# theOehrly/Formula-VAD

Measured on AMD Instinct MI355X. Metric: 48 kHz 480-sample VAD frames/sec whole node; max concurrent real-time streams, higher is better.
Workload: dtype f32

## Files before the change

formula-vad_amd/csrc/fvad_device.h:

```cpp
#pragma once
#pragma clang fp contract(off)
#include <hip/hip_runtime.h>

#include <cmath>

#include "fvad_internal.h"

namespace fvad {

constexpr float kWs = 1.f / 256;

__device__ __forceinline__ float2 cmul(float2 a, float2 b) {
  float2 m;
  m.x = a.x * b.x - a.y * b.y;
  m.y = a.x * b.y + a.y * b.x;
  return m;
}
__device__ __forceinline__ float2 cadd(float2 a, float2 b) { return make_float2(a.x + b.x, a.y + b.y); }
__device__ __forceinline__ float2 csub(float2 a, float2 b) { return make_float2(a.x - b.x, a.y - b.y); }

__device__ __forceinline__ float tansig(const float *__restrict__ table, float x) {
  if (!(x < 8)) return 1;
  if (!(x > -8)) return -1;
  if (x != x) return 0;
  float sign = 1;
  if (x < 0) {
    x = -x;
    sign = -1;
  }
  const int i = (int)floorf(.5f + 25 * x);
  x -= .04f * i;
  float y = table[i];
  const float dy = 1 - y * y;
  y = y + x * dy * (1 - y * x);
  return sign * y;
}
__device__ __forceinline__ float sigmoid(const float *__restrict__ table, float x) {
  return (float)(.5 + .5 * (double)tansig(table, (float)(.5 * (double)x)));
}
__device__ __forceinline__ float activate(const float *__restrict__ table, int act, float x) {
  if (act == kActSigmoid) return sigmoid(table, x);
  if (act == kActTanh) return tansig(table, x);
  return x < 0 ? 0 : x;
}

__device__ __forceinline__ void bfly4(float2 *F, int m, float2 tw1, float2 tw2, float2 tw3) {
  float2 a0 = F[0];
  const float2 s0 = cmul(F[m], tw1), s1 = cmul(F[2 * m], tw2), s2 = cmul(F[3 * m], tw3);
  const float2 s5 = csub(a0, s1);
  a0 = cadd(a0, s1);
  const float2 s3 = cadd(s0, s2), s4 = csub(s0, s2);
  F[2 * m] = csub(a0, s3);
  a0 = cadd(a0, s3);
  F[0] = a0;
  F[m] = make_float2(s5.x + s4.y, s5.y - s4.x);
  F[3 * m] = make_float2(s5.x - s4.y, s5.y + s4.x);
}

__device__ __forceinline__ void bfly3(float2 *F, int m, float2 tw1, float2 tw2, float2 epi3) {
  float2 a0 = F[0];
  const float2 s1 = cmul(F[m], tw1), s2 = cmul(F[2 * m], tw2);
  const float2 s3 = cadd(s1, s2);
  float2 s0 = csub(s1, s2);
  const float2 b1 = make_float2(a0.x - s3.x * .5f, a0.y - s3.y * .5f);
  s0.x *= epi3.y;
  s0.y *= epi3.y;
  a0 = cadd(a0, s3);
  F[0] = a0;
  F[2 * m] = make_float2(b1.x + s0.y, b1.y - s0.x);
  F[m] = make_float2(b1.x - s0.y, b1.y + s0.x);
}

__device__ __forceinline__ void kbfly5(float2 *F, int m, float2 t1, float2 t2, float2 t3, float2 t4, float2 ya,
                                       float2 yb) {
  const float2 s0 = F[0];
  const float2 s1 = cmul(F[m], t1), s2 = cmul(F[2 * m], t2), s3 = cmul(F[3 * m], t3), s4 = cmul(F[4 * m], t4);
  const float2 s7 = cadd(s1, s4), s10 = csub(s1, s4), s8 = cadd(s2, s3), s9 = csub(s2, s3);
  F[0] = make_float2(s0.x + (s7.x + s8.x), s0.y + (s7.y + s8.y));
  const float2 s5 = make_float2(s0.x + s7.x * ya.x + s8.x * yb.x, s0.y + s7.y * ya.x + s8.y * yb.x);
  const float2 s6 = make_float2(s10.y * ya.y + s9.y * yb.y, -(s10.x * ya.y) - s9.x * yb.y);
  F[m] = csub(s5, s6);
  F[4 * m] = cadd(s5, s6);
  const float2 s11 = make_float2(s0.x + s7.x * yb.x + s8.x * ya.x, s0.y + s7.y * yb.x + s8.y * ya.x);
  const float2 s12 = make_float2(-(s10.y * yb.y) + s9.y * ya.y, s10.x * yb.y - s9.x * ya.y);
  F[2 * m] = cadd(s11, s12);
  F[3 * m] = csub(s11, s12);
}

__device__ __forceinline__ void kiss_stage(float2 *W, float2 *S, int p, int m, int nc,
                                           const float2 *__restrict__ tw, int tid, int nt) {
  if (p == 1) return;
  const int fstride = nc / (p * m);
  if (p <= 5) {
    const int nb = fstride * m;
    for (int idx = tid; idx < nb; idx += nt) {
      const int g = idx / m, u = idx - g * m;
      float2 *F = W + g * p * m + u;
      if (p == 4) {
        bfly4(F, m, tw[u * fstride], tw[2 * u * fstride], tw[3 * u * fstride]);
      } else if (p == 2) {
        const float2 t = cmul(F[m], tw[u * fstride]);
        F[m] = csub(F[0], t);
        F[0] = cadd(F[0], t);
      } else if (p == 3) {
        bfly3(F, m, tw[u * fstride], tw[2 * u * fstride], tw[fstride * m]);
      } else {
        kbfly5(F, m, tw[u * fstride], tw[2 * u * fstride], tw[3 * u * fstride], tw[4 * u * fstride],
               tw[fstride * m], tw[fstride * 2 * m]);
      }
    }
    return;
  }
  const int no = fstride * m * p;
  for (int idx = tid; idx < no; idx += nt) {
    const int g = idx / (p * m), r = idx - g * (p * m), q1 = r / m, u = r - q1 * m;
    const float2 *F = W + g * p * m + u;
    const int k = u + q1 * m;
    float2 acc = F[0];
    int twidx = 0;
    for (int q = 1; q < p; q++) {
      twidx += fstride * k;
      if (twidx >= nc) twidx -= nc;
      acc = cadd(acc, cmul(F[q * m], tw[twidx]));
    }
    S[g * p * m + k] = acc;
  }
}

__device__ __forceinline__ void kiss_stages(float2 *W, float2 *S, const int *__restrict__ fac, int nf, int nc,
                                            const float2 *__restrict__ tw, int tid, int nt) {
  for (int k = nf - 1; k >= 0; k--) {
    const int p = fac[2 * k], m = fac[2 * k + 1];
    kiss_stage(W, S, p, m, nc, tw, tid, nt);
    __syncthreads();
    if (p > 5) {
      for (int i = tid; i < nc; i += nt) W[i] = S[i];
      __syncthreads();
    }
  }
}


__device__ __forceinline__ void bfly5(float2 *F, int m, float2 t1, float2 t2, float2 t3, float2 t4, float2 ya,
                                      float2 yb) {
  const float2 s0 = F[0];
  const float2 s1 = cmul(F[m], t1), s2 = cmul(F[2 * m], t2), s3 = cmul(F[3 * m], t3), s4 = cmul(F[4 * m], t4);
  const float2 s7 = cadd(s1, s4), s10 = csub(s1, s4), s8 = cadd(s2, s3), s9 = csub(s2, s3);
  float2 f0;
  f0.x = s0.x + (s7.x + s8.x);
  f0.y = s0.y + (s7.y + s8.y);
  float2 s5, s6, s11, s12;
  s5.x = s0.x + s7.x * ya.x + s8.x * yb.x;
  s5.y = s0.y + s7.y * ya.x + s8.y * yb.x;
  s6.x = s10.y * ya.y + s9.y * yb.y;
  s6.y = -(s10.x * ya.y) - s9.x * yb.y;
  s11.x = s0.x + s7.x * yb.x + s8.x * ya.x;
  s11.y = s0.y + s7.y * yb.x + s8.y * ya.x;
  s12.x = -(s10.y * yb.y) + s9.y * ya.y;
  s12.y = s10.x * yb.y - s9.x * ya.y;
  F[0] = f0;
  F[m] = csub(s5, s6);
  F[4 * m] = cadd(s5, s6);
  F[2 * m] = cadd(s11, s12);
  F[3 * m] = csub(s11, s12);
}

template <int NT>
__device__ void fft960_stages(float2 *W, const float2 *__restrict__ tw, int tid) {
  for (int b = tid; b < 240; b += NT) {
    float2 *F = W + 4 * b;
    float2 f0 = F[0];
    const float2 f1 = F[1], f2 = F[2], f3 = F[3];
    const float2 s0 = csub(f0, f2);
    f0 = cadd(f0, f2);
    float2 s1 = cadd(f1, f3);
    F[2] = csub(f0, s1);
    F[0] = cadd(f0, s1);
    s1 = csub(f1, f3);
    F[1] = make_float2(s0.x + s1.y, s0.y - s1.x);
    F[3] = make_float2(s0.x - s1.y, s0.y + s1.x);
  }
  __syncthreads();
  for (int q = tid; q < 240; q += NT) {
    const int i = q >> 2, j = q & 3;
    bfly4(W + i * 16 + j, 4, tw[j * 60], tw[j * 120], tw[j * 180]);
  }
  __syncthreads();
  for (int q = tid; q < 240; q += NT) {
    const int i = q >> 4, j = q & 15;
    bfly4(W + i * 64 + j, 16, tw[j * 15], tw[j * 30], tw[j * 45]);
  }
  __syncthreads();
  {
    const float2 epi3 = tw[320];
    for (int q = tid; q < 320; q += NT) {
      const int i = q >> 6, k = q & 63;
      bfly3(W + i * 192 + k, 64, tw[k * 5], tw[k * 10], epi3);
    }
  }
  __syncthreads();
  {
    const float2 ya = tw[192], yb = tw[384];
    for (int u = tid; u < 192; u += NT) bfly5(W + u, 192, tw[u], tw[2 * u], tw[3 * u], tw[4 * u], ya, yb);
  }
  __syncthreads();
}

struct Fft960Tw {
  float2 s2[3], s3[3], s4a[2], s4b[2], s5[4];
  float2 epi3, ya, yb;
};
__device__ __forceinline__ void fft960_load(Fft960Tw &t, const float2 *__restrict__ tw, int tid) {
  const int j2 = tid & 3, j3 = tid & 15, k4 = tid & 63;
  t.s2[0] = tw[j2 * 60];
  t.s2[1] = tw[j2 * 120];
  t.s2[2] = tw[j2 * 180];
  t.s3[0] = tw[j3 * 15];
  t.s3[1] = tw[j3 * 30];
  t.s3[2] = tw[j3 * 45];
  t.s4a[0] = tw[k4 * 5];
  t.s4a[1] = tw[k4 * 10];
  t.s4b[0] = t.s4a[0];
  t.s4b[1] = t.s4a[1];
  const int u = tid < 192 ? tid : 0;
  t.s5[0] = tw[u];
  t.s5[1] = tw[2 * u];
  t.s5[2] = tw[3 * u];
  t.s5[3] = tw[4 * u];
  t.epi3 = tw[320];
  t.ya = tw[192];
  t.yb = tw[384];
}
template <int F, int P>
__device__ __forceinline__ void fft960_run(const Fft960Tw &t, float2 (*W)[P], int tid) {
  if (tid < 240) {
#pragma unroll
    for (int fr = 0; fr < F; fr++) {
      float2 *Fp = W[fr] + 4 * tid;
      float2 f0 = Fp[0];
      const float2 f1 = Fp[1], f2 = Fp[2], f3 = Fp[3];
      const float2 s0 = csub(f0, f2);
      f0 = cadd(f0, f2);
      float2 s1 = cadd(f1, f3);
      Fp[2] = csub(f0, s1);
      Fp[0] = cadd(f0, s1);
      s1 = csub(f1, f3);
      Fp[1] = make_float2(s0.x + s1.y, s0.y - s1.x);
      Fp[3] = make_float2(s0.x - s1.y, s0.y + s1.x);
    }
  }
  __syncthreads();
  if (tid < 240) {
#pragma unroll
    for (int fr = 0; fr < F; fr++) bfly4(W[fr] + (tid >> 2) * 16 + (tid & 3), 4, t.s2[0], t.s2[1], t.s2[2]);
  }
  __syncthreads();
  if (tid < 240) {
#pragma unroll
    for (int fr = 0; fr < F; fr++) bfly4(W[fr] + (tid >> 4) * 64 + (tid & 15), 16, t.s3[0], t.s3[1], t.s3[2]);
  }
  __syncthreads();
#pragma unroll
  for (int fr = 0; fr < F; fr++) {
    bfly3(W[fr] + (tid >> 6) * 192 + (tid & 63), 64, t.s4a[0], t.s4a[1], t.epi3);
    if (tid < 64) bfly3(W[fr] + ((tid + 256) >> 6) * 192 + (tid & 63), 64, t.s4b[0], t.s4b[1], t.epi3);
  }
  __syncthreads();
  if (tid < 192) {
#pragma unroll
    for (int fr = 0; fr < F; fr++) bfly5(W[fr] + tid, 192, t.s5[0], t.s5[1], t.s5[2], t.s5[3], t.ya, t.yb);
  }
  __syncthreads();
}

struct BandEdges {
  float frac[400];
  int of[400];
  int e4[kBands + 2];
};
struct BandTab : BandEdges {
  float dct[kBands * kBands];
};
__device__ __forceinline__ void bandedges_load(BandEdges &b, const Plan *__restrict__ P, int tid, int nt) {
  for (int i = tid; i < 400; i += nt) {
    b.frac[i] = P->band_frac[i];
    b.of[i] = P->band_of[i];
  }
  for (int i = tid; i < kBands; i += nt) b.e4[i] = P->eband4[i];
}
__device__ __forceinline__ void bandtab_load(BandTab &b, const Plan *__restrict__ P, int tid, int nt) {
  bandedges_load(b, P, tid, nt);
  for (int i = tid; i < kBands * kBands; i += nt) b.dct[i] = P->dct[i];
}
__device__ __forceinline__ float band_sum_t(const float2 *A, const float2 *B, const BandEdges &T, int b) {
  float acc = 0;
  if (b >= 1) {
#pragma unroll 4
    for (int k = T.e4[b - 1]; k < T.e4[b]; k++) {
      float tmp = A[k].x * B[k].x;
      tmp += A[k].y * B[k].y;
      acc += T.frac[k] * tmp;
    }
  }
  if (b <= kBands - 2) {
#pragma unroll 4
    for (int k = T.e4[b]; k < T.e4[b + 1]; k++) {
      float tmp = A[k].x * B[k].x;
      tmp += A[k].y * B[k].y;
      acc += (1 - T.frac[k]) * tmp;
    }
  }
  if (b == 0 || b == kBands - 1) acc *= 2;
  return acc;
}
__device__ __forceinline__ void band_terms(float2 A, float2 B, const BandEdges &T, int k, float &lo, float &hi) {
  float tmp = A.x * B.x;
  tmp += A.y * B.y;
  hi = T.frac[k] * tmp;
  lo = (1 - T.frac[k]) * tmp;
}
__device__ __forceinline__ float band_chain(const float *lo, const float *hi, const BandEdges &T, int b) {
  float acc = 0;
  if (b >= 1) {
    const float4 *h4 = reinterpret_cast<const float4 *>(hi);
    for (int q = T.e4[b - 1] >> 2; q < T.e4[b] >> 2; q++) {
      const float4 v = h4[q];
      acc += v.x;
      acc += v.y;
      acc += v.z;
      acc += v.w;
    }
  }
  if (b <= kBands - 2) {
    const float4 *l4 = reinterpret_cast<const float4 *>(lo);
    for (int q = T.e4[b] >> 2; q < T.e4[b + 1] >> 2; q++) {
      const float4 v = l4[q];
      acc += v.x;
      acc += v.y;
      acc += v.z;
      acc += v.w;
    }
  }
  if (b == 0 || b == kBands - 1) acc *= 2;
  return acc;
}

__device__ __forceinline__ float interp_gain_t(const float *bandE, const BandEdges &T, int k) {
  if (k >= 400) return 0.0f;
  const int b = T.of[k];
  const float frac = T.frac[k];
  return (1 - frac) * bandE[b] + frac * bandE[b + 1];
}

__device__ __forceinline__ float band_sum(const float2 *A, const float2 *B, const Plan *__restrict__ P, int b) {
  float acc = 0;
  if (b >= 1) {
#pragma unroll 4
    for (int k = P->eband4[b - 1]; k < P->eband4[b]; k++) {
      float tmp = A[k].x * B[k].x;
      tmp += A[k].y * B[k].y;
      acc += P->band_frac[k] * tmp;
    }
  }
  if (b <= kBands - 2) {
#pragma unroll 4
    for (int k = P->eband4[b]; k < P->eband4[b + 1]; k++) {
      float tmp = A[k].x * B[k].x;
      tmp += A[k].y * B[k].y;
      acc += (1 - P->band_frac[k]) * tmp;
    }
  }
  if (b == 0 || b == kBands - 1) acc *= 2;
  return acc;
}

__device__ __forceinline__ float interp_gain(const float *bandE, const Plan *__restrict__ P, int k) {
  if (k >= 400) return 0.0f;
  const int b = P->band_of[k];
  const float frac = P->band_frac[k];
  return (1 - frac) * bandE[b] + frac * bandE[b + 1];
}

__device__ __forceinline__ float dot_seq(float acc, const float *a, int sa, const float *b, int sb, int n) {
  float a0[4], b0[4], a1[4], b1[4];
#pragma unroll
  for (int u = 0; u < 4; u++) {
    a0[u] = a[u * sa];
    b0[u] = b[u * sb];
    a1[u] = a[(4 + u) * sa];
    b1[u] = b[(4 + u) * sb];
  }
  int i = 0;
  for (; i + 8 < n; i += 4) {
    float a2[4], b2[4];
#pragma unroll
    for (int u = 0; u < 4; u++) {
      a2[u] = a[(i + 8 + u) * sa];
      b2[u] = b[(i + 8 + u) * sb];
    }
#pragma unroll
    for (int u = 0; u < 4; u++) acc = acc + a0[u] * b0[u];
#pragma unroll
    for (int u = 0; u < 4; u++) {
      a0[u] = a1[u];
      b0[u] = b1[u];
      a1[u] = a2[u];
      b1[u] = b2[u];
    }
  }
#pragma unroll
  for (int u = 0; u < 4; u++) acc = acc + a0[u] * b0[u];
#pragma unroll
  for (int u = 0; u < 4; u++) acc = acc + a1[u] * b1[u];
  return acc;
}

__device__ void syy_sequence(const float *y, int ys, int len, int max_pitch, float *syy) {
  float Syy = dot_seq(1.0f, y, ys, y, ys, len);
#pragma unroll 4
  for (int i = 0; i < max_pitch; i++) {
    syy[i] = Syy;
    const float ya = y[(i + len) * ys], yb = y[i * ys];
    Syy += ya * ya - yb * yb;
    Syy = (1 > Syy) ? 1 : Syy;
  }
}

__device__ __forceinline__ void best_pitch_visit(float xc, float Syy, int i, float &bn0, float &bn1, float &bd0,
                                                 float &bd1, int *best) {
  float xcorr16 = xc;
  xcorr16 *= 1e-12f;
  const float num = xcorr16 * xcorr16;
  const bool c1 = (xc > 0) && (num * bd1 > bn1 * Syy);
  const bool c2 = c1 && (num * bd0 > bn0 * Syy);
  bn1 = c2 ? bn0 : (c1 ? num : bn1);
  bd1 = c2 ? bd0 : (c1 ? Syy : bd1);
  best[1] = c2 ? best[0] : (c1 ? i : best[1]);
  bn0 = c2 ? num : bn0;
  bd0 = c2 ? Syy : bd0;
  best[0] = c2 ? i : best[0];
}

__device__ __forceinline__ float pitch_gain(float xy, float xx, float yy) { return xy / sqrtf(1 + xx * yy); }

__device__ __forceinline__ int second_check(int k) { return (int)((0x4d54d35534c0ull >> (3 * k)) & 7); }

template <int NT>
__device__ void dense_layer(const DevDense &d, const float *in, float *out, const float *tansig_tab, int tid) {
  for (int i = tid; i < d.nout; i += NT) {
    float sum = d.b[i];
#pragma unroll 8
    for (int j = 0; j < d.nin; j++) sum += d.w[j * d.nout + i] * in[j];
    out[i] = activate(tansig_tab, d.act, kWs * sum);
  }
}

template <int NT>
__device__ void gru_gates(const DevGru &g, const float *in, const float *state, float *zr, const float *tab,
                          int tid) {
  const int N = g.nout, M = g.nin, S3 = 3 * N;
  for (int t = tid; t < 2 * N; t += NT) {
    const int col = t;
    float sum = g.b[col];
#pragma unroll 8
    for (int j = 0; j < M; j++) sum += g.win[j * S3 + col] * in[j];
#pragma unroll 8
    for (int j = 0; j < N; j++) sum += g.wrec[j * S3 + col] * state[j];
    zr[t] = sigmoid(tab, kWs * sum);
  }
}
template <int NT>
__device__ void gru_out(const DevGru &g, const float *in, const float *state, const float *zr, float *h,
                        const float *tab, int tid) {
  const int N = g.nout, M = g.nin, S3 = 3 * N;
  for (int i = tid; i < N; i += NT) {
    float sum = g.b[2 * N + i];
#pragma unroll 8
    for (int j = 0; j < M; j++) sum += g.win[j * S3 + 2 * N + i] * in[j];
#pragma unroll 8
    for (int j = 0; j < N; j++) sum += g.wrec[j * S3 + 2 * N + i] * state[j] * zr[N + j];
    sum = activate(tab, g.act, kWs * sum);
    h[i] = zr[i] * state[i] + (1 - zr[i]) * sum;
  }
}


}
```

formula-vad_amd/csrc/fvad_internal.h:

```cpp
#pragma once
#include <cstddef>
#include <cstdint>

namespace fvad {

constexpr int kFrame = 480;
constexpr int kWin = 960;
constexpr int kFreq = 481;
constexpr int kBands = 22;
constexpr int kFeat = 42;
constexpr int kCeps = 8;
constexpr int kPitchBuf = 1728;
constexpr int kPitchMax = 768;
constexpr int kPitchMin = 60;
constexpr int kXlp = kPitchBuf / 2;
constexpr int kMaxNeurons = 128;
constexpr int kMaxCh = 8;
constexpr int kMaxBandCfg = 4;

constexpr int kMaxFftB = 16384;
constexpr int kMaxFftSize = 1 << 22;
constexpr int kMaxFactors = 32;

constexpr int windows_per_tick(int fft_size) { return fft_size >= kFrame ? 1 : (fft_size - 1 + kFrame) / fft_size; }

namespace st {
constexpr int kPitch = 0;
constexpr int kNdSamples = kPitch;
constexpr int kSyn = kPitch + kPitchBuf;
constexpr int kCepsMem = kSyn + kFrame;
constexpr int kLastG = kCepsMem + kCeps * kBands;
constexpr int kVadGru = kLastG + kBands;
constexpr int kNoiseGru = kVadGru + kMaxNeurons;
constexpr int kDenGru = kNoiseGru + kMaxNeurons;
constexpr int kHp = kDenGru + kMaxNeurons;
constexpr int kMemId = kHp + 2;
constexpr int kLastPeriod = kMemId + 1;
constexpr int kLastGain = kLastPeriod + 1;
constexpr int kFramesDone = kLastGain + 1;
constexpr int kVolAcc = kFramesDone + 1;
constexpr int kCepsDist = kVolAcc + 1;
constexpr int kWords = ((kCepsDist + kCeps * kCeps + 63) / 64) * 64;
}

namespace rnnimg {
constexpr int kMats = 9;
constexpr int kCols[kMats] = {24, 48, 24, 96, 48, 192, 96, 22, 1};
constexpr int kKin[kMats] = {42, 24, 24, 90, 90, 114, 114, 96, 24};
constexpr int kK[kMats] = {42, 48, 48, 138, 138, 210, 210, 96, 24};
constexpr int kSegs[kMats][4] = {{42, 0, 0, 0},   {24, 24, 0, 0},  {24, 24, 0, 0},
                                 {24, 24, 42, 48}, {24, 24, 42, 48}, {24, 48, 42, 96},
                                 {24, 48, 42, 96}, {96, 0, 0, 0},   {24, 0, 0, 0}};
constexpr int pad8(int x) { return (x + 7) & ~7; }
constexpr int pad16(int x) { return (x + 15) & ~15; }
constexpr int seg_off(int m, int g) {
  int o = 0;
  for (int i = 0; i < g; i++) o += pad8(kSegs[m][i]);
  return o;
}
constexpr int stride(int m) { return seg_off(m, 4); }
constexpr int off_b(int m) {
  int o = 0;
  for (int i = 0; i < m; i++) o += pad16(kCols[i]) + pad16(kCols[i] * stride(i));
  return o;
}
constexpr int off_w(int m) { return off_b(m) + pad16(kCols[m]); }
constexpr int kBytes = off_b(kMats);
}

struct Plan {
  float half_window[kFrame];
  float dct[kBands * kBands];
  float tansig[201];
  float band_frac[400];
  int band_of[400];
  int eband4[kBands];
  float tw960[2 * kWin];
  int bitrev960[kWin];
  int ibitrev960[kWin];
  int nfft_b;
  int ncfft_b;
  int stages_b;
  int nfac_b;
  int fac_b[2 * kMaxFactors];
  int generic_b;
  float norm_b;
  float twb[2 * kMaxFftB / 2];
  float superb[2 * kMaxFftB / 4];
  int permb[kMaxFftB / 2];
  float hannb[kMaxFftB];
};

struct DevDense {
  int nin, nout, act;
  const float *w;
  const float *b;
};
struct DevGru {
  int nin, nout, act;
  const float *win;
  const float *wrec;
  const float *b;
};
struct DevModel {
  DevDense in_dense, den_out, vad_out;
  DevGru vad, noise, den;
};

constexpr int kActTanh = 0, kActSigmoid = 1, kActRelu = 2;

struct HostLayer {
  int nin = 0, nout = 0, act = 0;
  bool gru = false;
  std::size_t off_w = 0, off_r = 0, off_b = 0;
};
struct HostModel {
  HostLayer layers[6];
  int8_t *blob = nullptr;
  std::size_t blob_size = 0;
};

void build_plan(Plan *p, int nfft_b);
float build_fftb_tables(int nfft_b, const int *fac, float *twb, float *superb, int *permb, float *hannb);

}

int fvad_synth_group(uint32_t base, int s0, int ns, int n_channels, int total_ticks, int tick0, int n_ticks,
                     float *out, std::size_t out_streams);
```

formula-vad_amd/csrc/fvad_plan.cpp:

```cpp
#include <cmath>
#include <cstdio>
#include <cstdlib>
#include <cstring>

#include "fvad_internal.h"

namespace fvad {
namespace {

const int kEband5ms[kBands] = {0, 1, 2, 3, 4, 5, 6, 7, 8, 10, 12, 14, 16, 20, 24, 28, 34, 40, 48, 60, 78, 100};

void celt_digit_reverse(int fout, int *f, int fstride, const int *factors) {
  const int p = factors[0], m = factors[1];
  if (m == 1) {
    for (int j = 0; j < p; j++) {
      *f = fout + j;
      f += fstride;
    }
  } else {
    for (int j = 0; j < p; j++) {
      celt_digit_reverse(fout, f, fstride * p, factors + 2);
      f += fstride;
      fout += m;
    }
  }
}

void kiss_factor(int n, int *fac, int *nf) {
  int p = 4, k = 0;
  const double floor_sqrt = std::floor(std::sqrt((double)n));
  do {
    while (n % p) {
      switch (p) {
        case 4: p = 2; break;
        case 2: p = 3; break;
        default: p += 2; break;
      }
      if (p > floor_sqrt) p = n;
    }
    n /= p;
    fac[2 * k] = p;
    fac[2 * k + 1] = n;
    k++;
  } while (n > 1);
  *nf = k;
}

void kiss_leaf_perm(int *perm, int out_base, int in_base, int fstride, const int *factors) {
  const int p = factors[0], m = factors[1];
  if (m == 1) {
    for (int j = 0; j < p; j++) perm[out_base + j] = in_base + j * fstride;
  } else {
    for (int j = 0; j < p; j++) kiss_leaf_perm(perm, out_base + j * m, in_base + j * fstride, fstride * p, factors + 2);
  }
}

}

void build_plan(Plan *p, int nfft_b) {
  std::memset(p, 0, sizeof(Plan));
  const double pi = 3.14159265358979323846;
  for (int i = 0; i < kFrame; i++) {
    const double s = std::sin(.5 * pi * (i + .5) / kFrame);
    p->half_window[i] = (float)std::sin(.5 * pi * s * s);
  }
  for (int i = 0; i < kBands; i++)
    for (int j = 0; j < kBands; j++) {
      float v = (float)std::cos((i + .5) * j * pi / kBands);
      if (j == 0) v = (float)(v * std::sqrt(.5));
      p->dct[i * kBands + j] = v;
    }
  for (int i = 0; i < 201; i++) {
    char buf[64];
    std::snprintf(buf, sizeof buf, "%f", std::tanh(0.04 * i));
    p->tansig[i] = std::strtof(buf, nullptr);
  }
  for (int b = 0; b < kBands; b++) p->eband4[b] = kEband5ms[b] << 2;
  for (int b = 0; b < kBands - 1; b++) {
    const int size = (kEband5ms[b + 1] - kEband5ms[b]) << 2;
    for (int j = 0; j < size; j++) {
      p->band_of[(kEband5ms[b] << 2) + j] = b;
      p->band_frac[(kEband5ms[b] << 2) + j] = (float)j / size;
    }
  }
  for (int i = 0; i < kWin; i++) {
    const double cpi = 3.14159265358979323846264338327;
    const double phase = (-2 * cpi / kWin) * i;
    p->tw960[2 * i] = (float)std::cos(phase);
    p->tw960[2 * i + 1] = (float)std::sin(phase);
  }
  const int celt_factors[10] = {5, 192, 3, 64, 4, 16, 4, 4, 4, 1};
  celt_digit_reverse(0, p->bitrev960, 1, celt_factors);
  for (int i = 0; i < kWin; i++) p->ibitrev960[p->bitrev960[i]] = i;
  p->nfft_b = nfft_b;
  p->ncfft_b = nfft_b / 2;
  const int nc = p->ncfft_b;
  kiss_factor(nc, p->fac_b, &p->nfac_b);
  int st = 0;
  for (int i = 0; i < p->nfac_b; i++) {
    st = (p->fac_b[2 * i] == 4 && st == i) ? st + 1 : st;
    if (p->fac_b[2 * i] > 5) p->generic_b = 1;
  }
  p->stages_b = st == p->nfac_b ? st : 0;
  if (nfft_b <= kMaxFftB) p->norm_b = build_fftb_tables(nfft_b, p->fac_b, p->twb, p->superb, p->permb, p->hannb);
}

float build_fftb_tables(int nfft_b, const int *fac, float *twb, float *superb, int *permb, float *hannb) {
  const double pi = 3.14159265358979323846;
  const int nc = nfft_b / 2;
  for (int i = 0; i < nc; i++) {
    const double kpi = 3.141592653589793238462643383279502884197169399375105820974944;
    const double phase = -2 * kpi * i / nc;
    twb[2 * i] = (float)std::cos(phase);
    twb[2 * i + 1] = (float)std::sin(phase);
  }
  for (int i = 0; i < nc / 2; i++) {
    const double phase = -3.14159265358979323846264338327 * ((double)(i + 1) / nc + .5);
    superb[2 * i] = (float)std::cos(phase);
    superb[2 * i + 1] = (float)std::sin(phase);
  }
  kiss_leaf_perm(permb, 0, 0, 1, fac);
  const float N = (float)nfft_b;
  const float two_pi = (float)(2.0 * pi);
  for (int i = 0; i < nfft_b; i++) {
    const float nn = (float)i;
    float acc = 0;
    for (int k = 0; k <= 1; k++) {
      const float kk = (float)k;
      const float sgn = k == 0 ? 1.0f : -1.0f;
      const float arg = ((two_pi * kk) * nn) / N;
      acc += (sgn * 0.5f) * (float)std::cos((double)arg);
    }
    hannb[i] = acc;
  }
  float sum = 0;
  for (int i = 0; i < nfft_b; i++) sum += hannb[i];
  const float window_norm = (float)nfft_b / sum;
  return window_norm / (float)(nfft_b / 2);
}

}
```

formula-vad_amd/csrc/fvad_wave.hip:

```cpp
#pragma clang fp contract(off)
#include <hip/hip_runtime.h>

#include <algorithm>
#include <cmath>

#include "fvad_device.h"
#include "fvad_internal.h"
#include "fvad_staged.h"
#include "fvad_staged_dev.h"
#include "fvad_wavedev.h"
#include "fvad_wfft.h"

namespace fvad {

constexpr int kWB = 8;
constexpr int kWNW = 4;
constexpr int kWOcc = 3;

constexpr int kWaveStatic = (1 << kWavePspec) | (1 << kWaveSynth);
__device__ __forceinline__ bool wave_is_static(const StagedArgs &, WaveKernel k) { return (kWaveStatic >> k) & 1; }
template <int NW = kWNW>
__device__ __forceinline__ long long wave_first(const StagedArgs &a, WaveKernel k, int slot, int lane) {
  return wave_is_static(a, k) ? (long long)blockIdx.x * NW + (threadIdx.x >> 6) : wave_take(a, slot, lane);
}
template <int NW = kWNW>
__device__ __forceinline__ long long wave_next(const StagedArgs &a, WaveKernel k, int slot, int lane, long long g) {
  return wave_is_static(a, k) ? g + (long long)gridDim.x * NW : wave_take(a, slot, lane);
}

__device__ __forceinline__ int batch_frames(const StagedArgs &a, long long g, int lane) {
  return lane < kWB ? frame_of(a, g, kWB, lane) : -1;
}
__device__ __forceinline__ int lane_val(int v, int l) { return __builtin_amdgcn_readlane(v, l); }
__device__ __forceinline__ void settle(int v) { asm volatile("" ::"v"(v)); }

__global__ void __launch_bounds__(64 * kWNW, kWOcc) k_fftAw(StagedArgs a) {
  __shared__ __attribute__((aligned(16))) float2 Rg[kWNW][wfft::kSlots];
  __shared__ WaveTabs tb;
  __shared__ float exb[kWNW][kWB][kBands + 2], lyb[kWNW][kWB][kBands + 2];
  __shared__ int silb[kWNW][kWB];
  const int tid = threadIdx.x, lane = tid & 63, wv = tid >> 6;
  wave_tabs_load(tb, a.plan, tid, 64 * kWNW);
  wfft::Tw tw;
  wfft::load_tw(tw, reinterpret_cast<const float2 *>(a.plan->tw960), lane);
  __syncthreads();
  const BandTab &T = tb.T;
  float2 *R = Rg[wv];
  float *tr = reinterpret_cast<float *>(R);
  const long long nb = ((long long)a.n_streams * a.V + kWB - 1) / kWB;
  for (long long g = wave_first(a, kWaveFftA, kWorkFftA, lane); g < nb; g = wave_next(a, kWaveFftA, kWorkFftA, lane, g)) {
    const int fl = batch_frames(a, g, lane);
    for (int fr = 0; fr < kWB; fr++) {
      const int f = lane_val(fl, fr);
      if (f < 0) continue;
      float2 v[16];
      const float *pb = frame_pb(a, f);
      static_assert(kXlp - kXlpHist == 4 * 60 && kHist % 4 == 0, "x_lp lanes");
      float xm = 0;
      float4 qa = make_float4(0, 0, 0, 0), qb = qa;
      if (lane < 60) {
        const float *q = pb + kHist + 8 * lane;
        xm = q[-1];
        qa = *reinterpret_cast<const float4 *>(q);
        qb = *reinterpret_cast<const float4 *>(q + 4);
      }
      WinRaw w;
      win_load(w, pb + (kPitchBuf - kWin), lane);
      win_apply(w, tb.hw, lane, v);
      wfft::run(v, tw, tb.tw, R, lane);
      float2 *X = a.X + (size_t)f * kFreq;
#pragma unroll
      for (int r = 0; r < 8; r++)
        if (64 * r + lane < kFreq) X[64 * r + lane] = v[r];
      if (lane < 60) {
        float4 o;
        o.x = xlp_value(xm, qa.x, qa.y);
        o.y = xlp_value(qa.y, qa.z, qa.w);
        o.z = xlp_value(qa.w, qb.x, qb.y);
        o.w = xlp_value(qb.y, qb.z, qb.w);
        *reinterpret_cast<float4 *>(frame_xlp(a, f) + kXlpHist + 4 * lane) = o;
      }
#pragma unroll
      for (int r = 0; r < 7; r++) {
        const int n = 64 * r + lane;
        if (n < 400) band_terms(v[r], v[r], T, n, tr[n], tr[400 + n]);
      }
      wfft::wsync();
      if (lane < kBands) {
        const float ex = band_chain(tr, tr + 400, T, lane);
        a.Ex[(size_t)f * kBands + lane] = ex;
        exb[wv][fr][lane] = ex;
        lyb[wv][fr][lane] = (float)log10(1e-2 + (double)ex);
      }
      wfft::wsync();
    }
    if (lane < kWB) {
      const int f = fl;
      if (f >= 0) {
        float *Ly = lyb[wv][lane];
        const float *Exl = exb[wv][lane];
        float logMax = -2, follow = -2, E = 0;
        for (int i = 0; i < kBands; i++) {
          const float ly0 = Ly[i];
          const double bb = (follow - 1.5 > (double)ly0) ? follow - 1.5 : (double)ly0;
          const double aa = ((double)(logMax - 7) > bb) ? (double)(logMax - 7) : bb;
          const float ly = (float)aa;
          Ly[i] = ly;
          logMax = (logMax > ly) ? logMax : ly;
          follow = (float)((follow - 1.5 > (double)ly) ? follow - 1.5 : (double)ly);
          E += Exl[i];
        }
        const int sil = ((double)E < 0.04) ? 1 : 0;
        silb[wv][lane] = sil;
        a.silence[f] = sil;
      }
    }
    wfft::wsync();
    for (int idx = lane; idx < kWB * kBands; idx += 64) {
      const int fr = idx / kBands, b = idx - fr * kBands;
      const int f = __shfl(fl, fr);
      if (f >= 0 && !silb[wv][fr]) {
        const float *Ly = lyb[wv][fr];
        float sum = 0;
#pragma unroll
        for (int j = 0; j < kBands; j++) sum += Ly[j] * T.dct[j * kBands + b];
        float val = (float)(sum * sqrt(2. / 22));
        if (b == 0) val -= 12;
        if (b == 1) val -= 4;
        a.Lyf[(size_t)f * kBands + b] = val;
      }
    }
    wfft::wsync();
  }
}

constexpr int kPNW = 8;
__global__ void __launch_bounds__(64 * kPNW, 4) k_pspecw(StagedArgs a) {
  __shared__ __attribute__((aligned(16))) float2 Rg[kPNW][wfft::kSlots];
  __shared__ WaveTabs tb;
  const int tid = threadIdx.x, lane = tid & 63, wv = tid >> 6;
  wave_tabs_load(tb, a.plan, tid, 64 * kPNW);
  wfft::Tw tw;
  wfft::load_tw(tw, reinterpret_cast<const float2 *>(a.plan->tw960), lane);
  __syncthreads();
  float2 *R = Rg[wv];
  const long long nb = ((long long)a.n_streams * a.V + kWB - 1) / kWB;
  for (long long g = wave_first<kPNW>(a, kWavePspec, kWorkPspec, lane); g < nb;
       g = wave_next<kPNW>(a, kWavePspec, kWorkPspec, lane, g)) {
    const int fl = batch_frames(a, g, lane);
    const int pl = fl >= 0 ? a.pitch[fl] : 0;
    settle(pl);
#pragma unroll 1
    for (int fr = 0; fr < kWB; fr++) {
      const int f = lane_val(fl, fr);
      if (f < 0) continue;
      const float v34 = pspec_frame(a, f, lane_val(pl, fr), tb, tw, R, lane);
      if (lane < 7) a.f34[(size_t)f * 8 + lane] = v34;
    }
  }
}

constexpr int kSNW = 8;
constexpr int kSOcc = 4;
struct SynthTabs {
  BandEdges T;
  wfft::TwTab tw;
  float hw[kFrame];
};
__global__ void __launch_bounds__(64 * kSNW, kSOcc) k_synthw(StagedArgs a) {
  __shared__ __attribute__((aligned(16))) float2 Rg[kSNW][wfft::kSlots];
  __shared__ SynthTabs tb;
  __shared__ float bp[kSNW][3][kBands + 2];
  const int tid = threadIdx.x, lane = tid & 63, wv = tid >> 6;
  bandedges_load(tb.T, a.plan, tid, 64 * kSNW);
  wfft::load_twtab(tb.tw, reinterpret_cast<const float2 *>(a.plan->tw960), tid, 64 * kSNW);
  for (int i = tid; i < kFrame; i += 64 * kSNW) tb.hw[i] = a.plan->half_window[i];
  wfft::Tw tw;
  wfft::load_tw(tw, reinterpret_cast<const float2 *>(a.plan->tw960), lane);
  __syncthreads();
  const BandEdges &T = tb.T;
  float2 *R = Rg[wv];
  float *tr = reinterpret_cast<float *>(R);
  float *rr = bp[wv][0], *nrm = bp[wv][1], *gsm = bp[wv][2];
  const long long nb = ((long long)a.n_streams * a.V + kWB - 1) / kWB;
  for (long long g = wave_first<kSNW>(a, kWaveSynth, kWorkSynth, lane); g < nb;
       g = wave_next<kSNW>(a, kWaveSynth, kWorkSynth, lane, g)) {
    const int fl = batch_frames(a, g, lane);
    const int sl = fl >= 0 ? a.silence[fl] : 0;
    settle(sl);
    for (int fr = 0; fr < kWB; fr++) {
      const int f = lane_val(fl, fr);
      if (f < 0) continue;
      const bool fil = !lane_val(sl, fr);
      const float2 *X = a.X + (size_t)f * kFreq;
      const float2 *P = a.P + (size_t)f * kFreq;
      float2 xv[8], pv[8];
#pragma unroll
      for (int r = 0; r < 8; r++) xv[r] = X[min(64 * r + lane, kFreq - 1)];
#pragma unroll
      for (int r = 0; r < 8; r++) pv[r] = P[min(64 * r + lane, kFreq - 1)];
      const size_t o = (size_t)f * kBands + min(lane, kBands - 1);
      const float Exp = a.Exp[o], Ex = a.Ex[o], Ep = a.Ep[o];
      const float gg = a.gr[o], gs = a.gs[o];
      if (fil) {
        if (lane < kBands) {
          float r;
          if (Exp > gg)
            r = 1;
          else
            r = (float)((double)((Exp * Exp) * (1 - (gg * gg))) / (.001 + (double)((gg * gg) * (1 - (Exp * Exp)))));
          float cl = (0 > r) ? 0 : r;
          cl = (1 < cl) ? 1 : cl;
          r = (float)sqrt((double)cl);
          r = (float)((double)r * sqrt((double)Ex / (1e-8 + (double)Ep)));
          rr[lane] = r;
          gsm[lane] = gs;
        }
        wfft::wsync();
#pragma unroll
        for (int r = 0; r < 8; r++) {
          const int n = 64 * r + lane;
          if (n < kFreq) {
            const float rf = interp_gain_t(rr, T, n);
            xv[r].x += rf * pv[r].x;
            xv[r].y += rf * pv[r].y;
            if (n < 400) band_terms(xv[r], xv[r], T, n, tr[n], tr[400 + n]);
          }
        }
        wfft::wsync();
        if (lane < kBands) {
          const float newE = band_chain(tr, tr + 400, T, lane);
          nrm[lane] = (float)sqrt((double)Ex / (1e-8 + (double)newE));
        }
        wfft::wsync();
#pragma unroll
        for (int r = 0; r < 8; r++) {
          const int n = 64 * r + lane;
          if (n < kFreq) {
            const float nf = interp_gain_t(nrm, T, n);
            xv[r].x *= nf;
            xv[r].y *= nf;
            const float gf = interp_gain_t(gsm, T, n);
            xv[r].x *= gf;
            xv[r].y *= gf;
          }
        }
      }
#pragma unroll
      for (int r = 0; r < 8; r++)
        if (64 * r + lane < kFreq) R[64 * r + lane] = xv[r];
      wfft::wsync();
      float2 v[16];
#pragma unroll
      for (int k = 0; k < 16; k++) {
        const int i = wfft::in_index(lane, k);
        float2 val = make_float2(0, 0);
        if (lane < 60) {
          if (i < kFreq) {
            val = R[i];
          } else {
            const float2 c = R[kWin - i];
            val = make_float2(c.x, -c.y);
          }
        }
        v[k] = make_float2(kScale960 * val.x, kScale960 * val.y);
      }
      wfft::wsync();
      wfft::run(v, tw, tb.tw, R, lane);
      float *y = a.ys + (size_t)f * kWin;
#pragma unroll
      for (int r = 0; r < 15; r++) {
        const int n = 64 * r + lane;
        const int i = (n == 0) ? 0 : kWin - n;
        const float yv = kWin * v[r].x;
        y[i] = yv * win960(tb.hw, i);
      }
      wfft::wsync();
    }
  }
}

constexpr int kFbSlots = 1040;
constexpr int kFbMag = 256;

struct FbTabs {
  float2 t4[4][3][16];
  float2 t5[4][3][64];
};

struct FbTw {
  float2 s2[4][3], s3[3], tw0;
};
__device__ __forceinline__ void fftb_tabs_load(FbTabs &tb, const Plan *__restrict__ P, int tid, int nt) {
  const float2 *__restrict__ twb = reinterpret_cast<const float2 *>(P->twb);
  for (int i = tid; i < 4 * 3 * 16; i += nt) {
    const int d2 = i / 48, r = (i / 16) % 3, u = i % 16;
    tb.t4[d2][r][u] = twb[4 * (r + 1) * (u + 16 * d2)];
  }
  for (int i = tid; i < 4 * 3 * 64; i += nt) {
    const int d3 = i / 192, r = (i / 64) % 3, l = i % 64;
    tb.t5[d3][r][l] = twb[(r + 1) * (l + 64 * d3)];
  }
}
__device__ __forceinline__ void fftb_tw_load(FbTw &w, const Plan *__restrict__ P, int lane) {
  const float2 *__restrict__ twb = reinterpret_cast<const float2 *>(P->twb) + opaque0();
#pragma unroll
  for (int d0 = 0; d0 < 4; d0++)
#pragma unroll
    for (int r = 0; r < 3; r++) w.s2[d0][r] = twb[64 * (r + 1) * d0];
#pragma unroll
  for (int r = 0; r < 3; r++) w.s3[r] = twb[16 * (r + 1) * (lane >> 2)];
  w.tw0 = twb[0];
}

__device__ __forceinline__ float fftb_bands(float2 (&v)[16], float2 *R, float *mag, const FbTabs &tb,
                                            const StagedArgs &a, int lane) {
  const Plan *__restrict__ P = a.plan;
  FbTw w;
  fftb_tw_load(w, P, lane);
  const float2 *__restrict__ sup = reinterpret_cast<const float2 *>(P->superb);
  const int nb = a.n_bands, lo = a.bin_lo_all, hi = a.bin_hi_all;
#pragma unroll
  for (int d1 = 0; d1 < 4; d1++) {
    float2 F[4] = {v[d1], v[d1 + 4], v[d1 + 8], v[d1 + 12]};
    bfly4(F, 1, w.tw0, w.tw0, w.tw0);
#pragma unroll
    for (int u = 0; u < 4; u++) v[d1 + 4 * u] = F[u];
  }
#pragma unroll
  for (int d0 = 0; d0 < 4; d0++) {
    float2 F[4] = {v[4 * d0], v[4 * d0 + 1], v[4 * d0 + 2], v[4 * d0 + 3]};
    bfly4(F, 1, w.s2[d0][0], w.s2[d0][1], w.s2[d0][2]);
#pragma unroll
    for (int u = 0; u < 4; u++) v[4 * d0 + u] = F[u];
  }
  wfft::wsync();
  {
    float2 *wr = R + (lane & 3) + 260 * ((lane >> 2) & 3) + 64 * (lane >> 4);
#pragma unroll
    for (int r = 0; r < 16; r++) wr[4 * (r >> 2) + 16 * (r & 3)] = v[r];
  }
  wfft::wsync();
  {
    const float2 *rd = R + lane;
#pragma unroll
    for (int r = 0; r < 16; r++) v[r] = rd[64 * (r & 3) + 260 * (r >> 2)];
  }
#pragma unroll
  for (int d3 = 0; d3 < 4; d3++) {
    float2 F[4] = {v[4 * d3], v[4 * d3 + 1], v[4 * d3 + 2], v[4 * d3 + 3]};
    bfly4(F, 1, w.s3[0], w.s3[1], w.s3[2]);
#pragma unroll
    for (int u = 0; u < 4; u++) v[4 * d3 + u] = F[u];
  }
#pragma unroll
  for (int d2 = 0; d2 < 4; d2++) {
    float2 F[4] = {v[d2], v[d2 + 4], v[d2 + 8], v[d2 + 12]};
    const int u16 = lane >> 2;
    bfly4(F, 1, tb.t4[d2][0][u16], tb.t4[d2][1][u16], tb.t4[d2][2][u16]);
#pragma unroll
    for (int u = 0; u < 4; u++) v[d2 + 4 * u] = F[u];
  }
  wfft::wsync();
  {
    float2 *wr = R + (lane >> 2) + 260 * (lane & 3);
#pragma unroll
    for (int r = 0; r < 16; r++) wr[16 * (r & 3) + 64 * (r >> 2)] = v[r];
  }
  wfft::wsync();
  {
    const float2 *rd = R + lane;
#pragma unroll
    for (int r = 0; r < 16; r++) v[r] = rd[64 * (r & 3) + 260 * (r >> 2)];
  }
#pragma unroll
  for (int d3 = 0; d3 < 4; d3++) {
    float2 F[4] = {v[d3], v[d3 + 4], v[d3 + 8], v[d3 + 12]};
    bfly4(F, 1, tb.t5[d3][0][lane], tb.t5[d3][1][lane], tb.t5[d3][2][lane]);
#pragma unroll
    for (int u = 0; u < 4; u++) v[d3 + 4 * u] = F[u];
  }
  wfft::wsync();
#pragma unroll
  for (int r = 0; r < 16; r++) R[64 * r + lane] = v[r];
  wfft::wsync();
  const int nc = 1024;
  for (int k = lo + lane; k <= hi; k += 64) {
    float re, imv;
    if (k == 0) {
      re = R[0].x + R[0].y;
      imv = 0;
    } else if (k == nc) {
      re = R[0].x - R[0].y;
      imv = 0;
    } else {
      const int kk = (k < nc / 2) ? k : nc - k;
      const float2 fpk = R[kk];
      const float2 fpnk = make_float2(R[nc - kk].x, -R[nc - kk].y);
      const float2 f1k = cadd(fpk, fpnk), f2k = csub(fpk, fpnk);
      const float2 tw2 = cmul(f2k, sup[kk - 1]);
      if (k < nc / 2) {
        re = (f1k.x + tw2.x) * ((float).5);
        imv = (f1k.y + tw2.y) * ((float).5);
      } else {
        re = (f1k.x - tw2.x) * ((float).5);
        imv = (tw2.y - f1k.y) * ((float).5);
      }
    }
    const float r2 = re * re, i2 = imv * imv;
    mag[k - lo] = sqrtf(r2 + i2) * P->norm_b;
  }
  wfft::wsync();
  float acc = 0.0f;
  if (lane < nb)
    for (int k = a.band_lo[lane]; k <= a.band_hi[lane]; k++) acc += mag[k - lo];
  wfft::wsync();
  return acc;
}

__global__ void __launch_bounds__(64 * kWNW, kWOcc) k_fftbw(StagedArgs a) {
  __shared__ __attribute__((aligned(16))) float2 Rg[kWNW][kFbSlots];
  __shared__ float mg[kWNW][kFbMag];
  __shared__ FbTabs tb;
  const int tid = threadIdx.x, lane = tid & 63, wv = tid >> 6;
  const Plan *__restrict__ P = a.plan;
  fftb_tabs_load(tb, P, tid, 64 * kWNW);
  __syncthreads();
  float2 *R = Rg[wv];
  float *mag = mg[wv];
  const int C = a.n_channels, nb = a.n_bands;
  const long long items = (long long)a.n_streams * a.wmax * C;
  const long long nw = (long long)gridDim.x * kWNW;
  for (long long it = (long long)blockIdx.x * kWNW + wv; it < items; it += nw) {
    const int c = (int)(it % C);
    const long long sj = it / C;
    const int s = (int)(sj / a.wmax), j = (int)(sj - (long long)s * a.wmax);
    const int t = a.win_tick[(size_t)s * a.wmax + j];
    if (t < 0) continue;
    const long long wstart = a.win_start[(size_t)s * a.wmax + j];
    const float *ring = a.ring + ((size_t)s * C + c) * a.ring_len;
    const int rl = a.ring_len, w0 = (int)(wstart % rl);
    float2 v[16];
#pragma unroll
    for (int r = 0; r < 16; r++) {
      const int k = lane + 64 * r;
      int i0 = w0 + 2 * k;
      i0 -= (i0 >= rl) ? rl : 0;
      int i1 = i0 + 1;
      i1 -= (i1 >= rl) ? rl : 0;
      const float t0 = ring[i0] * P->hannb[2 * k];
      const float t1 = ring[i1] * P->hannb[2 * k + 1];
      v[r] = make_float2(t0, t1);
    }
    const float band = fftb_bands(v, R, mag, tb, a, lane);
    if (lane < nb) a.out_band[(((size_t)t * a.n_streams + s) * C + c) * nb + lane] = band;
  }
}

__global__ void __launch_bounds__(64 * kWNW, kWOcc) k_olafb(StagedArgs a) {
  __shared__ __attribute__((aligned(16))) float2 Rg[kWNW][kFbSlots];
  __shared__ float mg[kWNW][kFbMag];
  __shared__ float ovg[kWNW][kFrame];
  __shared__ FbTabs tb;
  const int tid = threadIdx.x, lane = tid & 63, wv = tid >> 6;
  const Plan *__restrict__ P = a.plan;
  fftb_tabs_load(tb, P, tid, 64 * kWNW);
  __syncthreads();
  constexpr int FB = 2048;
  float *ov = ovg[wv];
  static_assert(kFbSlots * 2 >= FB, "window fits the exchange region");
  float2 *R = Rg[wv];
  float *W = reinterpret_cast<float *>(R);
  float *mag = mg[wv];
  const int C = a.n_channels, nb = a.n_bands, B = a.n_streams, V = a.V;
  const int G = kWNW / C;
  const int wvu = __builtin_amdgcn_readfirstlane(wv);
  const int sw = wvu / C, c = wvu - sw * C;
  const float kInv = a.raw_s16 ? 1.0f : 1.0f / (float)32767;
  const int rl = a.ring_len;
  for (int sb = blockIdx.x * G; sb < B; sb += gridDim.x * G) {
    const int s = sb + sw;
    const bool on = sw < G && s < B;
    const int nt = __builtin_amdgcn_readfirstlane(on ? ticks_of(a, s) : 0);
    float *stp = a.state + (size_t)(on ? s : 0) * st::kWords;
    int fd0 = 0;
    float vol = 0;
    if (nt > 0) {
      fd0 = __builtin_amdgcn_readfirstlane(reinterpret_cast<const int *>(stp)[st::kFramesDone]);
      vol = __int_as_float(__builtin_amdgcn_readfirstlane(__float_as_int(stp[st::kVolAcc])));
    }
    long long ws = (long long)fd0 * kFrame / FB * FB;
    const float *ring = a.ring + ((size_t)(on ? s : 0) * C + c) * rl;
    if (nt > 0) {
      const int ncarry = (int)((long long)fd0 * kFrame - ws);
      const int r0 = (int)(ws % rl);
      for (int i = lane; i < ncarry; i += 64) {
        int ri = r0 + i;
        ri -= ri >= rl ? rl : 0;
        W[i] = ring[ri];
      }
    }
    __syncthreads();
    if (nt > 0) {
      const float *ysr = a.ys + (size_t)s * V * kWin;
      const bool sl = lane < 60;
      const int q = 8 * lane;
      auto load = [&](int t, float4 (&cur)[2], float4 (&prv)[2]) {
        const int v = t * C + c;
        const float *cp = ysr + (size_t)v * kWin + q;
        const float *pp = v == 0 ? stp + st::kSyn + q : ysr + (size_t)(v - 1) * kWin + kFrame + q;
        if (sl) {
          cur[0] = *reinterpret_cast<const float4 *>(cp);
          cur[1] = *reinterpret_cast<const float4 *>(cp + 4);
          prv[0] = *reinterpret_cast<const float4 *>(pp);
          prv[1] = *reinterpret_cast<const float4 *>(pp + 4);
        }
      };
      float4 cn[2] = {}, pn[2] = {};
      load(0, cn, pn);
      float tk_ratio = 0, tk_vad = 1;
      for (int t = 0; t < nt; t++) {
        if ((t & 63) == 0) {
          const int tl = t + lane;
          tk_ratio = 0;
          tk_vad = 1;
          if (tl < nt) {
            tk_ratio = a.ratio[(size_t)tl * B + s];
            for (int cc = 0; cc < C; cc++) {
              const float vv = a.vadf[(size_t)s * V + tl * C + cc];
              if (vv < tk_vad) tk_vad = vv;
            }
          }
        }
        float4 cur[2] = {cn[0], cn[1]}, prv[2] = {pn[0], pn[1]};
        const long long p0 = (long long)(fd0 + t) * kFrame;
        const int off = (int)(p0 - ws);
        const bool complete = off + kFrame >= FB;
        if (!complete && t + 1 < nt) load(t + 1, cn, pn);
        float o[8];
        o[0] = (cur[0].x + prv[0].x) * kInv;
        o[1] = (cur[0].y + prv[0].y) * kInv;
        o[2] = (cur[0].z + prv[0].z) * kInv;
        o[3] = (cur[0].w + prv[0].w) * kInv;
        o[4] = (cur[1].x + prv[1].x) * kInv;
        o[5] = (cur[1].y + prv[1].y) * kInv;
        o[6] = (cur[1].z + prv[1].z) * kInv;
        o[7] = (cur[1].w + prv[1].w) * kInv;
        const size_t ot = (size_t)t * B + s;
        if (a.out_den && sl) {
          float4 *dp = reinterpret_cast<float4 *>(a.out_den + (ot * C + c) * kFrame + q);
          dp[0] = make_float4(o[0], o[1], o[2], o[3]);
          dp[1] = make_float4(o[4], o[5], o[6], o[7]);
        }
        if (sl) {
#pragma unroll
          for (int e = 0; e < 8; e++)
            if (off + q + e < FB) W[off + q + e] = o[e];
        }
        const float vad_low = __int_as_float(__builtin_amdgcn_readlane(__float_as_int(tk_vad), t & 63));
        const float ratio = __int_as_float(__builtin_amdgcn_readlane(__float_as_int(tk_ratio), t & 63));
        if (complete) {
          const int r = FB - off;
          vol += ratio * ((float)r / (float)FB);
          if (c == 0 && lane == 0) {
            a.out_win_ratio[ot] = vol;
            a.out_win_vad[ot] = vad_low;
          }
          vol = 0;
          if (kFrame - r > 0) vol += ratio * ((float)(kFrame - r) / (float)FB);
          if (sl) {
#pragma unroll
            for (int e = 0; e < 8; e++)
              if (off + q + e >= FB) ov[off + q + e - FB] = o[e];
          }
          wfft::wsync();
          float2 v[16];
#pragma unroll
          for (int rr = 0; rr < 16; rr++) {
            const int k = lane + 64 * rr;
            const float2 x = *reinterpret_cast<const float2 *>(W + 2 * k);
            v[rr] = make_float2(x.x * P->hannb[2 * k], x.y * P->hannb[2 * k + 1]);
          }
          const float band = fftb_bands(v, R, mag, tb, a, lane);
          if (lane < nb) a.out_band[(ot * C + c) * nb + lane] = band;
          for (int i = lane; i < off + kFrame - FB; i += 64) W[i] = ov[i];
          ws += FB;
          if (t + 1 < nt) load(t + 1, cn, pn);
        } else {
          vol += ratio * ((float)kFrame / (float)FB);
          if (c == 0 && lane == 0) {
            a.out_win_ratio[ot] = 0.0f;
            a.out_win_vad[ot] = 0.0f;
          }
          if (lane < nb) a.out_band[(ot * C + c) * nb + lane] = 0.0f;
        }
        if (c == 0 && lane == 0) {
          a.out_vad[ot] = vad_low;
          a.out_win_flag[ot] = complete ? 1 : 0;
        }
      }
      wfft::wsync();
      const int ncarry = (int)((long long)(fd0 + nt) * kFrame - ws);
      const int r0 = (int)(ws % rl);
      float *rw = a.ring + ((size_t)s * C + c) * rl;
      for (int i = lane; i < ncarry; i += 64) {
        int ri = r0 + i;
        ri -= ri >= rl ? rl : 0;
        rw[ri] = W[i];
      }
    }
    __syncthreads();
    if (nt > 0) {
      if (c == 0 && lane == 0) {
        reinterpret_cast<int *>(stp)[st::kFramesDone] = fd0 + nt;
        stp[st::kVolAcc] = vol;
      }
      if (c == C - 1) {
        const float4 *yl =
            reinterpret_cast<const float4 *>(a.ys + ((size_t)s * V + (size_t)nt * C - 1) * kWin + kFrame);
        float4 *dst = reinterpret_cast<float4 *>(stp + st::kSyn);
        for (int i = lane; i < kFrame / 4; i += 64) dst[i] = yl[i];
      }
    }
  }
}

namespace {
template <typename K>
int wave_per_cu(K kernel, int nw = kWNW) {
  int per_cu = 0;
  if (hipOccupancyMaxActiveBlocksPerMultiprocessor(&per_cu, kernel, 64 * nw, 0) != hipSuccess || per_cu < 1)
    per_cu = 1;
  return per_cu;
}
}

hipError_t launch_wave(WaveKernel which, const StagedArgs &a, int n_cu, hipStream_t stream) {
  static const int p_fftA = wave_per_cu(k_fftAw), p_pspec = wave_per_cu(k_pspecw, kPNW), p_synth = wave_per_cu(k_synthw, kSNW),
                   p_fftb = wave_per_cu(k_fftbw), p_olafb = wave_per_cu(k_olafb);
  const int g_fftA = p_fftA * n_cu, g_pspec = p_pspec * n_cu, g_synth = p_synth * n_cu, g_fftb = p_fftb * n_cu,
            g_olafb = std::min(p_olafb, 2) * n_cu;
  if (which == kWaveOlaFb) {
    const int G = kWNW / a.n_channels;
    hipLaunchKernelGGL(k_olafb, dim3((unsigned)std::min<long long>((a.n_streams + G - 1) / G, g_olafb)), dim3(64 * kWNW),
                       0, stream, a);
    return hipGetLastError();
  }
  if (which == kWaveFftB) {
    const long long items = (long long)a.n_streams * a.wmax * a.n_channels;
    hipLaunchKernelGGL(k_fftbw, dim3((unsigned)std::min<long long>(std::max<long long>((items + kWNW - 1) / kWNW, 1), g_fftb)),
                       dim3(64 * kWNW), 0, stream, a);
    return hipGetLastError();
  }
  const long long batches = ((long long)a.n_streams * a.V + kWB - 1) / kWB;
  auto grid = [&](int resident, int nw = kWNW) {
    const long long want = ((kWaveStatic >> which) & 1) ? (batches + nw - 1) / nw : batches;
    return dim3((unsigned)std::min<long long>(std::max<long long>(want, 1), resident));
  };
  if (which == kWaveFftA)
    hipLaunchKernelGGL(k_fftAw, grid(g_fftA), dim3(64 * kWNW), 0, stream, a);
  else if (which == kWavePspec)
    hipLaunchKernelGGL(k_pspecw, grid(g_pspec, kPNW), dim3(64 * kPNW), 0, stream, a);
  else
    hipLaunchKernelGGL(k_synthw, grid(g_synth, kSNW), dim3(64 * kSNW), 0, stream, a);
  return hipGetLastError();
}

}
```

Before: 44.23 million.

## Pair frames for band-energy chains and prefetch chain loads in fftA kernel

The fftA wave kernel now processes frames two at a time. It stashes the first frame's band terms in registers and writes both frames' terms to the scratch buffer together, so one wave sync covers two frames. Lanes 0-21 and 32-53 then compute the two frames' band-energy chains at once, using a new fixed-length chain routine that prefetches float4 blocks three ahead and masks out unused blocks. The log10 of band energy is moved out of the per-frame loop into one pass over the whole batch. In exchange, each frame iteration holds more registers and runs a fixed 44-block loop instead of the exact band length.

```diff
diff --git a/formula-vad_amd/csrc/fvad_device.h b/formula-vad_amd/csrc/fvad_device.h
--- a/formula-vad_amd/csrc/fvad_device.h
+++ b/formula-vad_amd/csrc/fvad_device.h
@@ -344,6 +344,33 @@
   if (b == 0 || b == kBands - 1) acc *= 2;
   return acc;
 }
+constexpr int kChainAhead = 3;
+__device__ __forceinline__ void chain_hold(float &acc) { asm volatile("" : "+v"(acc) : : "memory"); }
+__device__ __forceinline__ float band_chain_ahead(const float *lo, const float *hi, const BandEdges &T, int b) {
+  const int qa = T.e4[b >= 1 ? b - 1 : 0] >> 2, qb = T.e4[b] >> 2, qc = T.e4[b <= kBands - 2 ? b + 1 : b] >> 2;
+  const int nh = qb - qa, nl = qc - qb;
+  const float4 *h4 = reinterpret_cast<const float4 *>(hi) + qa;
+  const float4 *l4 = reinterpret_cast<const float4 *>(lo) + (b <= kBands - 2 ? qb : 0);
+  float4 v[kChainAhead];
+#pragma unroll
+  for (int s = 0; s < kChainAhead; s++) v[s] = h4[s];
+  float acc = 0;
+#pragma unroll
+  for (int s = 0; s < 2 * kChainBlocks; s++) {
+    const float4 c = v[s % kChainAhead];
+    const bool mine = s < kChainBlocks ? s < nh : s - kChainBlocks < nl;
+    chain_hold(acc);
+    float t = acc + c.x;
+    t += c.y;
+    t += c.z;
+    t += c.w;
+    acc = mine ? t : acc;
+    const int n = s + kChainAhead;
+    if (n < 2 * kChainBlocks) v[s % kChainAhead] = n < kChainBlocks ? h4[n] : l4[n - kChainBlocks];
+  }
+  if (b == 0 || b == kBands - 1) acc *= 2;
+  return acc;
+}
 
 __device__ __forceinline__ float interp_gain_t(const float *bandE, const BandEdges &T, int k) {
   if (k >= 400) return 0.0f;
diff --git a/formula-vad_amd/csrc/fvad_internal.h b/formula-vad_amd/csrc/fvad_internal.h
--- a/formula-vad_amd/csrc/fvad_internal.h
+++ b/formula-vad_amd/csrc/fvad_internal.h
@@ -8,6 +8,7 @@
 constexpr int kWin = 960;
 constexpr int kFreq = 481;
 constexpr int kBands = 22;
+constexpr int kChainBlocks = 22;
 constexpr int kFeat = 42;
 constexpr int kCeps = 8;
 constexpr int kPitchBuf = 1728;
diff --git a/formula-vad_amd/csrc/fvad_plan.cpp b/formula-vad_amd/csrc/fvad_plan.cpp
--- a/formula-vad_amd/csrc/fvad_plan.cpp
+++ b/formula-vad_amd/csrc/fvad_plan.cpp
@@ -8,7 +8,14 @@
 namespace fvad {
 namespace {
 
-const int kEband5ms[kBands] = {0, 1, 2, 3, 4, 5, 6, 7, 8, 10, 12, 14, 16, 20, 24, 28, 34, 40, 48, 60, 78, 100};
+constexpr int kEband5ms[kBands] = {0, 1, 2, 3, 4, 5, 6, 7, 8, 10, 12, 14, 16, 20, 24, 28, 34, 40, 48, 60, 78, 100};
+
+constexpr bool chain_blocks_ok() {
+  for (int b = 0; b + 1 < kBands; b++)
+    if (kEband5ms[b + 1] - kEband5ms[b] > kChainBlocks || kEband5ms[b] + kChainBlocks > kEband5ms[kBands - 1]) return false;
+  return kEband5ms[0] == 0 && kEband5ms[kBands - 1] == 100;
+}
+static_assert(chain_blocks_ok(), "band table vs kChainBlocks");
 
 void celt_digit_reverse(int fout, int *f, int fstride, const int *factors) {
   const int p = factors[0], m = factors[1];
diff --git a/formula-vad_amd/csrc/fvad_wave.hip b/formula-vad_amd/csrc/fvad_wave.hip
--- a/formula-vad_amd/csrc/fvad_wave.hip
+++ b/formula-vad_amd/csrc/fvad_wave.hip
@@ -33,6 +33,43 @@
 }
 __device__ __forceinline__ int lane_val(int v, int l) { return __builtin_amdgcn_readlane(v, l); }
 __device__ __forceinline__ void settle(int v) { asm volatile("" ::"v"(v)); }
+
+__device__ __forceinline__ void fftA_frame(const StagedArgs &a, int f, const WaveTabs &tb, const wfft::Tw &tw, float2 *R,
+                                           int lane, float (&tl)[7], float (&th)[7]) {
+  float2 v[16];
+  const float *pb = frame_pb(a, f);
+  static_assert(kXlp - kXlpHist == 4 * 60 && kHist % 4 == 0, "x_lp lanes");
+  float xm = 0;
+  float4 qa = make_float4(0, 0, 0, 0), qb = qa;
+  if (lane < 60) {
+    const float *q = pb + kHist + 8 * lane;
+    xm = q[-1];
+    qa = *reinterpret_cast<const float4 *>(q);
+    qb = *reinterpret_cast<const float4 *>(q + 4);
+  }
+  WinRaw w;
+  win_load(w, pb + (kPitchBuf - kWin), lane);
+  win_apply(w, tb.hw, lane, v);
+  wfft::run(v, tw, tb.tw, R, lane);
+  float2 *X = a.X + (size_t)f * kFreq;
+#pragma unroll
+  for (int r = 0; r < 8; r++)
+    if (64 * r + lane < kFreq) X[64 * r + lane] = v[r];
+  if (lane < 60) {
+    float4 o;
+    o.x = xlp_value(xm, qa.x, qa.y);
+    o.y = xlp_value(qa.y, qa.z, qa.w);
+    o.z = xlp_value(qa.w, qb.x, qb.y);
+    o.w = xlp_value(qb.y, qb.z, qb.w);
+    *reinterpret_cast<float4 *>(frame_xlp(a, f) + kXlpHist + 4 * lane) = o;
+  }
+#pragma unroll
+  for (int r = 0; r < 7; r++) {
+    const int n = 64 * r + lane;
+    tl[r] = th[r] = 0;
+    if (n < 400) band_terms(v[r], v[r], tb.T, n, tl[r], th[r]);
+  }
+}
 
 __global__ void __launch_bounds__(64 * kWNW, kWOcc) k_fftAw(StagedArgs a) {
   __shared__ __attribute__((aligned(16))) float2 Rg[kWNW][wfft::kSlots];
@@ -50,50 +87,54 @@
   const long long nb = ((long long)a.n_streams * a.V + kWB - 1) / kWB;
   for (long long g = wave_first(a, kWaveFftA, kWorkFftA, lane); g < nb; g = wave_next(a, kWaveFftA, kWorkFftA, lane, g)) {
     const int fl = batch_frames(a, g, lane);
-    for (int fr = 0; fr < kWB; fr++) {
-      const int f = lane_val(fl, fr);
-      if (f < 0) continue;
-      float2 v[16];
-      const float *pb = frame_pb(a, f);
-      static_assert(kXlp - kXlpHist == 4 * 60 && kHist % 4 == 0, "x_lp lanes");
-      float xm = 0;
-      float4 qa = make_float4(0, 0, 0, 0), qb = qa;
-      if (lane < 60) {
-        const float *q = pb + kHist + 8 * lane;
-        xm = q[-1];
-        qa = *reinterpret_cast<const float4 *>(q);
-        qb = *reinterpret_cast<const float4 *>(q + 4);
-      }
-      WinRaw w;
-      win_load(w, pb + (kPitchBuf - kWin), lane);
-      win_apply(w, tb.hw, lane, v);
-      wfft::run(v, tw, tb.tw, R, lane);
-      float2 *X = a.X + (size_t)f * kFreq;
-#pragma unroll
-      for (int r = 0; r < 8; r++)
-        if (64 * r + lane < kFreq) X[64 * r + lane] = v[r];
-      if (lane < 60) {
-        float4 o;
-        o.x = xlp_value(xm, qa.x, qa.y);
-        o.y = xlp_value(qa.y, qa.z, qa.w);
-        o.z = xlp_value(qa.w, qb.x, qb.y);
-        o.w = xlp_value(qb.y, qb.z, qb.w);
-        *reinterpret_cast<float4 *>(frame_xlp(a, f) + kXlpHist + 4 * lane) = o;
-      }
-#pragma unroll
-      for (int r = 0; r < 7; r++) {
-        const int n = 64 * r + lane;
-        if (n < 400) band_terms(v[r], v[r], T, n, tr[n], tr[400 + n]);
+    unsigned todo = (unsigned)__builtin_amdgcn_ballot_w64(fl >= 0);
+    while (todo) {
+      const int fr0 = __builtin_ctz(todo);
+      todo &= todo - 1;
+      const int np = todo ? 2 : 1;
+      const int fr1 = todo ? __builtin_ctz(todo) : fr0;
+      todo &= todo - 1;
+      const int f0 = lane_val(fl, fr0), f1 = lane_val(fl, fr1);
+      float kl[7] = {}, kh[7] = {};
+#pragma unroll 1
+      for (int h = 0; h < np; h++) {
+        float tl[7], th[7];
+        fftA_frame(a, h ? f1 : f0, tb, tw, R, lane, tl, th);
+        if (h + 1 < np) {
+#pragma unroll
+          for (int r = 0; r < 7; r++) {
+            kl[r] = tl[r];
+            kh[r] = th[r];
+          }
+        } else {
+#pragma unroll
+          for (int r = 0; r < 7; r++) {
+            const int n = 64 * r + lane;
+            if (n < 400) {
+              if (h) {
+                tr[n] = kl[r];
+                tr[400 + n] = kh[r];
+              }
+              tr[800 * h + n] = tl[r];
+              tr[800 * h + 400 + n] = th[r];
+            }
+          }
+        }
       }
       wfft::wsync();
-      if (lane < kBands) {
-        const float ex = band_chain(tr, tr + 400, T, lane);
-        a.Ex[(size_t)f * kBands + lane] = ex;
-        exb[wv][fr][lane] = ex;
-        lyb[wv][fr][lane] = (float)log10(1e-2 + (double)ex);
+      const int h = lane >> 5, b = lane & 31;
+      if (b < kBands && h < np) {
+        const float ex = band_chain_ahead(tr + 800 * h, tr + 800 * h + 400, T, b);
+        a.Ex[(size_t)(h ? f1 : f0) * kBands + b] = ex;
+        exb[wv][h ? fr1 : fr0][b] = ex;
       }
       wfft::wsync();
     }
+    for (int idx = lane; idx < kWB * kBands; idx += 64) {
+      const int fr = idx / kBands, b = idx - fr * kBands;
+      if (__shfl(fl, fr) >= 0) lyb[wv][fr][b] = (float)log10(1e-2 + (double)exb[wv][fr][b]);
+    }
+    wfft::wsync();
     if (lane < kWB) {
       const int f = fl;
       if (f >= 0) {
```

New measurement: 44.92 million (median of 6 runs). +1.6%, better.
